# cornellius-gp/linear_operator

Measured on AMD Instinct MI355X. Metric: cg_member_matvecs_per_sec, higher is better.
Workload: dtype f32

## Files before the change

### linear_operator_amd/csrc/lo_rspace3.hip

```cpp
#include <algorithm>
#include <atomic>
#include <mutex>
#include <type_traits>
#include <stdlib.h>

#include "lo_device.h"
#include "lo_internal.h"
#include "lo_cg_onchip.h"
#include "lo_group_reduce.h"
#include "lo_cg_close.h"
#include "lo_f64_lanes.h"

namespace lo {

namespace {

typedef float f32x4 __attribute__((ext_vector_type(4)));
typedef __attribute__((address_space(1))) const f32x4 g_cf4;
typedef __attribute__((address_space(1))) const float g_cf;
typedef __attribute__((address_space(1))) float g_f;
typedef __attribute__((address_space(1))) const char g_cc;
template <class T>
__device__ __forceinline__ T* opaque_uniform(T* p) {
  asm volatile("" : "+s"(p));
  return p;
}

constexpr int R3_TPB = 256;
constexpr int R3_ROWS = 1024;

struct PeerOut {
  float* buf[7];
  int n;
  long long member_off;
};
PeerOut g_peer_out = {{nullptr, nullptr, nullptr, nullptr, nullptr, nullptr, nullptr}, 0, 0};
std::mutex g_peer_mu;

__host__ __device__ constexpr int r3_np(int RC) { return 2 * RC + 6; }

__device__ __forceinline__ unsigned xor4_dpp_u(unsigned x) {
  const int a = __builtin_amdgcn_update_dpp(0, (int)x, 0x104, 0xf, 0x5, false);
  return (unsigned)__builtin_amdgcn_update_dpp(a, (int)x, 0x114, 0xf, 0xa, false);
}
__device__ __forceinline__ double halve4_d(double lo, double hi, int lane) {
  const bool up = (lane & 4) != 0;
  const double keep = up ? hi : lo;
  const double send = up ? lo : hi;
  return keep + mk_d(xor4_dpp_u(lo_w(send)), xor4_dpp_u(hi_w(send)));
}

template <int CH>
__device__ __forceinline__ double rows_reduce_d(double (&p)[CH], int lane) {
  if constexpr (CH == 8) {
#pragma unroll
    for (int m = 0; m < 4; ++m) p[m] = halve4_d(p[m], p[m + 4], lane);
    p[0] = halve_pair_d<2>(p[0], p[2], lane);
    p[1] = halve_pair_d<2>(p[1], p[3], lane);
    return halve_pair_d<1>(p[0], p[1], lane);
  } else if constexpr (CH == 4) {
    p[0] = halve_pair_d<2>(p[0], p[2], lane);
    p[1] = halve_pair_d<2>(p[1], p[3], lane);
    return halve_pair_d<1>(p[0], p[1], lane);
  } else {
    return halve_pair_d<1>(p[0], p[1], lane);
  }
}

template <int RC, int GW>
__global__ __launch_bounds__(R3_TPB, 2) void k_cg_rspace3(OnchipArgs a, PeerOut po) {
  constexpr int CH = RC / 4;
  constexpr int RPI = 64 / CH;
  constexpr int NI = 256 / RPI;
  constexpr int NP = r3_np(RC);
  constexpr int MLD = RC + 2;
  constexpr int NH = RC / 2;
  constexpr int NG = 2 * GW * NP;
  __shared__ __attribute__((aligned(16))) float bst[4][256];
  __shared__ __attribute__((aligned(16))) float dst[4][256];
  __shared__ __attribute__((aligned(16))) double mat_s[3 * RC * MLD];
  __shared__ __attribute__((aligned(16))) double red[4][NP];
  __shared__ __attribute__((aligned(16))) double res[NP];
  __shared__ __attribute__((aligned(16))) double gv[4][32];
  __shared__ unsigned polw[GW > 1 ? NG : 2];
  const GroupPlace gp = group_place(GW, (int)gridDim.x / 8);
  if (!gp.active) return;
  const int grp = gp.grp, wig = gp.wig, ngroups = gp.ngroups;
  const int t = threadIdx.x, lane = t & 63, wave = t >> 6;
  const int wave_u = __builtin_amdgcn_readfirstlane(wave);
  unsigned long long* const gbase = a.gbuf + (size_t)grp * 2 * NG;
  unsigned tag = a.tag_base;
  bool same_xcd = false;
  const unsigned xcc = xcc_id();
  bool first = true;
  const int row0 = wig * R3_ROWS + 256 * wave_u;
  const int row0c = max(0, min(row0, a.N - 256));
  const bool di_full = a.dinv_mode == LO_DIAG_FULL;
  float* const bw = bst[wave_u];
  float* const dw = dst[wave_u];
  constexpr int NPF = 8;
  f32x4 pre[NPF];
  constexpr int NXT = NI - NPF;
  f32x4 nxt[NXT > 0 ? NXT : 1];
  auto request = [&](int64_t bm, int tl_, int i_lo, auto cnt, f32x4* dst) {
    const int ln_ = tl_ & 63, k_ = ln_ & (CH - 1), g_ = ln_ / CH;
    const unsigned loff = (unsigned)((g_ * RC + 4 * k_) * sizeof(float));
    g_cc* Cw = (g_cc*)(a.C + ((size_t)bm * a.N + row0c) * RC);
#pragma unroll
    for (int q = 0; q < decltype(cnt)::value / 8; ++q) {
      g_cc* bq = opaque_uniform(Cw + (i_lo + 8 * q + 4) * 1024);
#pragma unroll
      for (int i = 0; i < 8; ++i) dst[8 * q + i] = *(g_cf4*)(bq + loff + (i - 4) * 1024);
    }
  };
  int64_t b = grp;
  {
    int tl0 = t;
    asm volatile("" : "+v"(tl0));
    if (b < a.B) {
      request(b, tl0, 0, std::integral_constant<int, NPF>{}, pre);
      request(b, tl0, NPF, std::integral_constant<int, NXT>{}, nxt);
    } else {
#pragma unroll
      for (int i = 0; i < NPF; ++i) pre[i] = (f32x4){0.f, 0.f, 0.f, 0.f};
    }
  }
  while (b < a.B) {
    const bool stamp = a.dbg && b == a.dbg_member && wig == 0 && t == 0;
    if (stamp) a.dbg[0] = wall_clock64();
    int drawn = 0;
    if (wig == 0 && t == 0) drawn = atomicAdd(a.next_member, 1);
    int tl = t;
    asm volatile("" : "+v"(tl));
    const int ln = tl & 63, k = ln & (CH - 1), g = ln / CH;
    f32x4 Cr[NI];
#pragma unroll
    for (int i = 0; i < NPF; ++i) Cr[i] = pre[i];
#pragma unroll
    for (int i = 0; i < NXT; ++i) Cr[NPF + i] = nxt[i];
    float bq4[4], dq4[4];
    {
      g_cf* bb_ = opaque_uniform((g_cf*)(a.rhs + (size_t)b * a.N + row0c));
      g_cf* dd_ = opaque_uniform((g_cf*)(di_full ? a.dinv + (size_t)b * a.N + row0c : a.dinv + b));
      const int lo_e = row0 - row0c, hi_e = max(0, min(256, a.N - row0c));
      const int dstride = di_full ? 1 : 0;
#pragma unroll
      for (int m = 0; m < 4; ++m) {
        const int e = ln + 64 * m;
        const bool own = e >= lo_e && e < hi_e;
        bq4[m] = own ? bb_[e] : 0.f;
        dq4[m] = own ? dd_[e * dstride] : 0.f;
      }
    }
    constexpr int NM = (3 * RC * RC / 2 + R3_TPB - 1) / R3_TPB;
    f32x4 mv[NM];
    {
      typedef __attribute__((address_space(1))) const f32x4 g_m4;
      const g_m4* src = (const g_m4*)(a.RSD + (size_t)b * 6 * RC * RC);
#pragma unroll
      for (int u = 0; u < NM; ++u) {
        const int e = min(tl + R3_TPB * u, 3 * RC * RC / 2 - 1);
        const int ms = e / (RC * RC / 2);
        const int mg = ms == 0 ? 0 : ms + 1;
        mv[u] = src[(size_t)mg * (RC * RC / 2) + (e - ms * (RC * RC / 2))];
      }
    }
    const double lam_mine = a.RSD[((size_t)b * 6 + 5) * RC * RC + min(ln & 31, RC - 1)];
#pragma unroll
    for (int m = 0; m < 4; ++m) {
      bw[ln + 64 * m] = bq4[m];
      dw[ln + 64 * m] = dq4[m];
    }
#pragma unroll
    for (int u = 0; u < NM; ++u) {
      const int e = tl + R3_TPB * u;
      if (e < 3 * RC * RC / 2) {
        const int mi = e / (RC / 2), jj = e % (RC / 2);
        *reinterpret_cast<f32x4*>(&mat_s[mi * MLD + 2 * jj]) = mv[u];
      }
    }
    __builtin_amdgcn_wave_barrier();
    if (stamp) a.dbg[1] = wall_clock64();

    {
      double aw[4] = {0.0, 0.0, 0.0, 0.0}, au[4] = {0.0, 0.0, 0.0, 0.0};
#pragma unroll
      for (int i0 = 0; i0 < NI; i0 += 4) {
#pragma unroll
        for (int i = i0; i < i0 + 4; ++i) {
          const int r = RPI * i + g;
          const double bb = (double)bw[r];
          const double bd = bb * (double)dw[r];
          const double c0 = (double)Cr[i].x, c1 = (double)Cr[i].y, c2 = (double)Cr[i].z, c3 = (double)Cr[i].w;
          aw[0] = fma(c0, bd, aw[0]); au[0] = fma(c0, bb, au[0]);
          aw[1] = fma(c1, bd, aw[1]); au[1] = fma(c1, bb, au[1]);
          aw[2] = fma(c2, bd, aw[2]); au[2] = fma(c2, bb, au[2]);
          aw[3] = fma(c3, bd, aw[3]); au[3] = fma(c3, bb, au[3]);
        }
        __builtin_amdgcn_sched_barrier(0);
      }
      double s_acc = 0.0, a_acc = 0.0, d2_acc = 0.0;
#pragma unroll
      for (int j = 0; j < 4; ++j) {
        const int rw = 64 * j + RPI * k + g;
        const double bb = (double)bw[rw], di = (double)dw[rw];
        s_acc = fma(bb, bb * di, s_acc);
        a_acc = fma(bb, bb, a_acc);
        d2_acc = fma(di, di, d2_acc);
      }
      double h0 = halve_pair_d<32>(aw[0], au[0], ln), h1 = halve_pair_d<32>(aw[1], au[1], ln);
      double h2 = halve_pair_d<32>(aw[2], au[2], ln), h3 = halve_pair_d<32>(aw[3], au[3], ln);
      h0 = halve_pair_d<16>(h0, h2, ln);
      h1 = halve_pair_d<16>(h1, h3, ln);
      double mine = halve_pair_d<8>(h0, h1, ln);
      if constexpr (CH <= 4) mine = bfly_add_d<4>(mine);
      if constexpr (CH <= 2) mine = bfly_add_d<2>(mine);
      const int comp = (((ln >> 4) & 1) << 1) | ((ln >> 3) & 1);
      const bool writer = (ln & 7 & ~(CH - 1)) == 0;
      if (writer) red[wave_u][((ln >> 5) ? RC : 0) + 4 * k + comp] = mine;
      const double ssum = wave_sum_fast_d(s_acc), asum = wave_sum_fast_d(a_acc), d2sum = wave_sum_fast_d(d2_acc);
      if (ln == 0) {
        red[wave_u][2 * RC] = ssum;
        red[wave_u][2 * RC + 1] = asum;
        red[wave_u][2 * RC + 2] = (wig == 0 && wave_u == 0) ? (double)(ngroups + drawn) : 0.0;
        red[wave_u][2 * RC + 3] = d2sum;
        unsigned xc = xcc;
        asm volatile("" : "+s"(xc));
        red[wave_u][2 * RC + 4] = (first && wave_u == 0) ? (double)xc : 0.0;
        red[wave_u][2 * RC + 5] = (first && wave_u == 0) ? (double)(xc * xc) : 0.0;
      }
    }
#pragma unroll
    for (int i = 0; i < NI; ++i) asm volatile("" : "+v"(Cr[i]));
    __builtin_amdgcn_sched_barrier(0);
    if (a.prefetch & 4) __builtin_amdgcn_s_setprio(3);
    {
      ++tag;
      int tt = (int)threadIdx.x;
      asm volatile("" : "+v"(tt));
      __syncthreads();
      if constexpr (GW == 1) {
        if (tt < NP) res[tt] = (red[0][tt] + red[1][tt]) + (red[2][tt] + red[3][tt]);
      } else {
        unsigned long long* slot = gbase + (size_t)(tag & 1u) * NG;
        if (tt < NP) {
          const double v = (red[0][tt] + red[1][tt]) + (red[2][tt] + red[3][tt]);
          unsigned long long* mine = slot + ((size_t)wig * NP + tt) * 2;
          granule_store(mine, granule_pack_bits(tag, lo_w(v)), same_xcd);
          granule_store(mine + 1, granule_pack_bits(tag, hi_w(v)), same_xcd);
        }
        constexpr int PER = (NG + R3_TPB - 1) / R3_TPB;
        constexpr int CKQ = PER < 8 ? PER : 8;
        unsigned spin = 0;
        bool lost = false;
#pragma unroll 1
        for (int q0 = 0; q0 < PER && !lost; q0 += CKQ) {
          unsigned long long x[CKQ];
          for (;;) {
            bool ok = true;
#pragma unroll
            for (int q = 0; q < CKQ; ++q) {
              const int idx = tt + R3_TPB * (q0 + q);
              x[q] = granule_load(slot + min(idx, NG - 1));
              ok = ok && (granule_tag(x[q]) == tag);
            }
            if (ok) break;
            if (poll_give_up(spin, a.err)) {
              lost = true;
              break;
            }
            __builtin_amdgcn_s_sleep(1);
          }
#pragma unroll
          for (int q = 0; q < CKQ; ++q) {
            const int idx = tt + R3_TPB * (q0 + q);
            if (idx < NG) polw[idx] = granule_bits(x[q]);
          }
        }
        __syncthreads();
        if (tt < NP) {
          double tot = 0.0;
#pragma unroll
          for (int w = 0; w < GW; ++w) tot += mk_d(polw[(w * NP + tt) * 2], polw[(w * NP + tt) * 2 + 1]);
          res[tt] = tot;
        }
      }
      __syncthreads();
    }
    if (GW > 1 && first) {
      unsigned xc = xcc;
      asm volatile("" : "+s"(xc));
      same_xcd = same_xcd_verdict(res[2 * RC + 4], res[2 * RC + 5], GW, xc, a.allow_l2_handoff);
    }
    first = false;
    if (stamp) a.dbg[2] = wall_clock64();
    const int64_t b_next = (int64_t)res[2 * RC + 2];
    {
      int tp = t;
      asm volatile("" : "+v"(tp));
      if (b_next < a.B) {
        request(b_next, tp, 0, std::integral_constant<int, NPF>{}, pre);
      } else {
#pragma unroll
        for (int i = 0; i < NPF; ++i) pre[i] = (f32x4){0.f, 0.f, 0.f, 0.f};
      }
    }
    if (a.prefetch & 1) __builtin_amdgcn_s_setprio(3);

    const int j = lane & 31, hf = lane >> 5;
    const bool live = j < RC;
    const int jr = live ? j : RC - 1;
    double yj = 0.0, xi = 0.0;
    float nrm;
    {
      double a0 = res[2 * RC + 1], s = res[2 * RC];
      const double d2 = res[2 * RC + 3];
      nrm = sqrtf((float)a0);
      const bool rhs_zero = nrm < a.eps;
      if (rhs_zero) nrm = 1.0f;
      const double inv = 1.0 / (double)nrm;
      const double w0 = live ? res[jr] * inv : 0.0, u0 = live ? res[RC + jr] * inv : 0.0;
      s *= inv * inv;
      a0 *= inv * inv;
      float sa = a.stop_after;
      asm volatile("" : "+s"(sa));
      const double sure_rz = 2.0 * (double)sa * (double)sa * sqrt(d2);
      auto own_row_dot = [&](const double* mrow, const double* vec) {
        double a0_ = 0.0, a1_ = 0.0;
#pragma unroll
        for (int q = 0; q < NH; q += 2) {
          const double2 xa = *reinterpret_cast<const double2*>(mrow + q);
          const double2 xx = *reinterpret_cast<const double2*>(vec + q);
          a0_ = fma(xa.x, xx.x, a0_);
          a1_ = fma(xa.y, xx.y, a1_);
        }
        double lo_, up_;
        halves_d(a0_ + a1_, lo_, up_);
        return lo_ + up_;
      };
      double* myv = gv[wave];
      if (hf == 0) myv[j] = w0;
      __builtin_amdgcn_wave_barrier();
      const double* row0m = mat_s + (size_t)jr * MLD + hf * NH;
      double c0 = own_row_dot(row0m, myv + hf * NH);
      double e0 = own_row_dot(row0m + (size_t)1 * RC * MLD, myv + hf * NH);
      const double* nrow = row0m + (size_t)2 * RC * MLD;
      const double* tucol = mat_s + (size_t)(1 * RC + hf * NH) * MLD + jr;
      c0 = live ? c0 : 0.0;
      e0 = live ? e0 : 0.0;
      double tau2 = s - lanes32_sum_d(c0 * e0);
      tau2 = tau2 > 0.0 ? tau2 : 0.0;
      const bool delicate = !rhs_zero && tau2 < 1e-2 * s;
      const double lam = live ? lam_mine : 1.0;
      long long ts_a = 0, ts_b = 0;
      if (stamp) ts_a = wall_clock64();
      double cj = c0, qj = 0.0, etaj = 0.0;
      double cp = 1.0, qp = 0.0, etap = 0.0;
      double rz = 0.0, pApE = 0.0, alpha = 0.0, beta = 0.0;
      float rn = 0.f, last_alpha = 0.f;
      bool conv = false;
      unsigned close_flags = 0u;
      const size_t bc = (size_t)b;
      const bool rec = wig == 0 && lane == 0;
      const int last_owner = (a.iters - 1) & 3;
      for (int kk = -1; kk < a.iters; ++kk) {
        if (kk >= 0) {
          last_alpha = (float)alpha;
          etaj = fma(alpha, qj, etaj);
          etap = fma(alpha, qp, etap);
          cj = fma(-alpha * lam, qj, cj);
          cp = fma(-alpha, qp, cp);
        }
        const double lc = lam * cj;
        const bool lo_h = hf == 0;
        const float inv_rz = __builtin_amdgcn_rcpf((float)rz);
        const double red2 = row16_sum_d(halve_pair_d<16>(lo_h ? cj * cj : lc * qj, lo_h ? lc * cj : 0.0, lane));
        const auto pick = [&](double v, int ln_) {
          return mk_d((unsigned)__builtin_amdgcn_readlane((int)lo_w(v), ln_),
                      (unsigned)__builtin_amdgcn_readlane((int)hi_w(v), ln_));
        };
        const double cc = pick(red2, 0), clc = pick(red2, 16), clq = pick(red2, 32);
        const double rzn = fma(cp * cp, tau2, cc);
        const bool sure = rzn > sure_rz;
        const bool rec_first = kk == 0 && a.close_gran == nullptr && wave == 0;
        const bool rec_last = kk == a.iters - 1 && wave == last_owner;
        const bool own = rec_first || rec_last || !sure;
        float rnn = 0.f;
        if (kk < 0) {
          const float s1f = (float)a0;
          rnn = __builtin_amdgcn_sqrtf(s1f < 0.f ? 0.f : s1f);
        } else if (own) {
          const double dl = fma(-cp, c0, cj);
          __builtin_amdgcn_wave_barrier();
          if (hf == 0) myv[j] = dl;
          __builtin_amdgcn_wave_barrier();
          double gj_;
          {
            double a0_ = 0.0, a1_ = 0.0;
#pragma unroll
            for (int q = 0; q < NH; q += 2) {
              const double2 dd = *reinterpret_cast<const double2*>(myv + hf * NH + q);
              a0_ = fma(tucol[(size_t)q * MLD], dd.x, a0_);
              a1_ = fma(tucol[(size_t)(q + 1) * MLD], dd.y, a1_);
            }
            double lo_, up_;
            halves_d(a0_ + a1_, lo_, up_);
            gj_ = live ? lo_ + up_ : 0.0;
          }
          __builtin_amdgcn_wave_barrier();
          if (hf == 0) myv[j] = gj_;
          __builtin_amdgcn_wave_barrier();
          const double nd = own_row_dot(nrow, myv + hf * NH);
          const double r2 = row16_sum_d(halve_pair_d<16>(gj_ * nd, gj_ * u0, lane));
          const double dnd = pick(r2, 0), dm = pick(r2, 16);
          const double s1 = fma(cp, fma(cp, a0, 2.0 * dm), dnd);
          const float s1f = (float)s1;
          rnn = __builtin_amdgcn_sqrtf(s1f < 0.f ? 0.f : s1f);
        }
        if (kk >= 0) {
          beta = ((float)rz < a.eps) ? 0.0 : (double)((float)rzn * inv_rz);
          if (rhs_zero) rnn = 0.f;
          rn = rnn;
          if (rec && (rec_first || rec_last)) a.resid_rec[(size_t)kk * a.B + bc] = rn;
        } else {
          beta = 0.0;
          rn = rnn;
          if (wig == 0 && t == 0) a.init_conv[bc] = (rn < a.stop_after) ? 1 : 0;
          close_flags = ((rn < a.stop_after) ? 1u : 0u) | (delicate ? 4u : 0u);
          if (delicate && rec && wave == 0) atomicOr(a.err + 4, 1);
        }
        if (kk == 0 && (rnn != rnn || rzn != rzn)) close_flags |= 2u;
        conv = (own || rhs_zero) ? (rn < a.stop_after) : false;
        rz = rzn;
        pApE = fma(beta, fma(beta, pApE, 2.0 * clq), clc);
        qj = fma(beta, qj, cj);
        qp = fma(beta, qp, cp);
        const double pAp = fma(qp * qp, tau2, pApE);
        alpha = ((float)pAp < a.eps) ? 0.0 : (double)((float)rz * __builtin_amdgcn_rcpf((float)pAp));
        if (conv) alpha = 0.0;
      }
      if (stamp) ts_b = wall_clock64();
      if (rec && wave == last_owner) {
        a.rhs_norm[bc] = nrm;
        a.rhs_is_zero[bc] = rhs_zero ? 1 : 0;
        a.rz[bc] = (float)rz;
        a.alpha[bc] = last_alpha;
        a.beta[bc] = (float)beta;
        a.resid_norm[bc] = rn;
        a.has_conv[bc] = conv ? 1 : 0;
        if (a.close_gran) {
          granule_store(a.close_gran + b, granule_pack(a.close_epoch | close_flags, rn), false);
        }
      }
      __builtin_amdgcn_wave_barrier();
      if (hf == 0) myv[j] = fma(-etap, e0, etaj);
      __builtin_amdgcn_wave_barrier();
      xi = etap;
      {
        const double* col = mat_s + (size_t)(hf * NH) * MLD + jr;
        double a0_ = 0.0, a1_ = 0.0;
#pragma unroll
        for (int q = 0; q < NH; q += 2) {
          const double2 ee = *reinterpret_cast<const double2*>(myv + hf * NH + q);
          a0_ = fma(col[(size_t)q * MLD], ee.x, a0_);
          a1_ = fma(col[(size_t)(q + 1) * MLD], ee.y, a1_);
        }
        double lo_, up_;
        halves_d(a0_ + a1_, lo_, up_);
        yj = lo_ + up_;
      }
      yj = live ? yj : 0.0;
      if (stamp) {
        a.dbg[5] = ts_a - a.dbg[2];
        a.dbg[6] = ts_b - ts_a;
        a.dbg[7] = wall_clock64() - ts_b;
      }
      __builtin_amdgcn_wave_barrier();
      if (hf == 0) myv[j] = yj * (double)nrm;
      __builtin_amdgcn_wave_barrier();
    }
    if (!(a.prefetch & 2)) __builtin_amdgcn_s_setprio(0);
    if (stamp) a.dbg[3] = wall_clock64();
    {
      int l2 = lane;
      asm volatile("" : "+v"(l2));
      const int k2 = l2 & (CH - 1), g2 = l2 / CH;
      const double* myv = gv[wave];
      const double2 ya = *reinterpret_cast<const double2*>(&myv[4 * k2]);
      const double2 yb = *reinterpret_cast<const double2*>(&myv[4 * k2 + 2]);
      g_f* const xb = opaque_uniform((g_f*)(a.xout + (size_t)b * a.N + row0c));
      const bool more = b_next < a.B;
      g_cc* const Cn = (g_cc*)(a.C + ((size_t)(more ? b_next : b) * a.N + row0c) * RC);
      const unsigned loffn = (unsigned)((g2 * RC + 4 * k2) * sizeof(float));
#pragma unroll
      for (int js = 0; js < 4; ++js) {
        constexpr int J0 = NPF / CH;
        const int jj = (js + J0) & 3;
        double p[CH];
#pragma unroll
        for (int m = 0; m < CH; ++m) {
          const f32x4 c4 = Cr[CH * jj + m];
          p[m] = fma((double)c4.w, yb.y, fma((double)c4.z, yb.x, fma((double)c4.y, ya.y, (double)c4.x * ya.x)));
        }
        const double xv = rows_reduce_d<CH>(p, l2);
        const int rw = 64 * jj + RPI * k2 + g2;
        const int row = row0c + rw;
        const double acc = fma(xi, (double)bw[rw], xv);
        if (row >= row0 && row < a.N) {
          const float xval = (float)(acc * (double)dw[rw]);
          xb[rw] = xval;
          for (int pp = 0; pp < po.n; ++pp)
            ((g_f*)po.buf[pp])[((size_t)(b + po.member_off)) * a.N + row] = xval;
        }
        if (CH * jj >= NPF) {
          g_cc* bqn = opaque_uniform(Cn + (CH * jj + 4) * 1024);
#pragma unroll
          for (int m = 0; m < CH; ++m)
            nxt[CH * jj - NPF + m] = more ? *(g_cf4*)(bqn + loffn + (m - 4) * 1024) : (f32x4){0.f, 0.f, 0.f, 0.f};
        }
      }
      __builtin_amdgcn_wave_barrier();
    }
    __builtin_amdgcn_s_setprio(0);
    if (stamp) a.dbg[4] = wall_clock64();
    __syncthreads();
    b = b_next;
  }
  if (a.close_gran && wig == 0) cg_close_solve(a, ngroups, t);
}

int rspace3_prio() {
  static const int prio = [] {
    const char* e = getenv("LO_RS_PRIO");
    return e ? atoi(e) : 3;
  }();
  return prio;
}

constexpr size_t HO_MAX_WGS = 2 * 320;
constexpr size_t HO_GRAN_PER_WG = 432;
constexpr size_t HO_MAX_MEMBERS = 65536;
constexpr size_t HO_HEAD_BYTES = 256;
constexpr unsigned HO_TAG_LIMIT = 0xfff00000u;
constexpr unsigned HO_EPOCH_LIMIT = 0x1ffffff0u;
struct HandoffBlock {
  char* buf = nullptr;
  size_t bytes = 0;
  bool failed = false;
  unsigned next_tag = 1, next_epoch = 1;
  unsigned last_launch = 0;
  std::atomic<unsigned> confirmed{0};
  bool force_clear = false;
  unsigned clears = 0, launches = 0;
};
HandoffBlock g_handoff[16];
std::atomic<unsigned> g_handoff_ids{0};

HandoffBlock* handoff_block() {
  int dev = 0;
  if (hipGetDevice(&dev) != hipSuccess || dev < 0 || dev >= 16) return nullptr;
  HandoffBlock& h = g_handoff[dev];
  if (!h.buf && !h.failed) {
    h.bytes = HO_HEAD_BYTES + (HO_MAX_WGS * HO_GRAN_PER_WG + HO_MAX_MEMBERS) * sizeof(unsigned long long);
    if (hipMalloc(&h.buf, h.bytes) != hipSuccess || hipMemset(h.buf, 0, h.bytes) != hipSuccess) {
      (void)hipGetLastError();
      h.buf = nullptr;
      h.failed = true;
    }
  }
  return h.buf ? &h : nullptr;
}

bool handoff_advance(unsigned* next_tag, unsigned* next_epoch, int64_t B, unsigned* tag_base, unsigned* epoch) {
  bool wrap = false;
  const unsigned need = (unsigned)B + 2u;
  if (*next_tag >= HO_TAG_LIMIT - need || *next_epoch >= HO_EPOCH_LIMIT) {
    *next_tag = 1;
    *next_epoch = 1;
    wrap = true;
  }
  *tag_base = *next_tag;
  *epoch = *next_epoch;
  *next_tag += need;
  *next_epoch += 1;
  return wrap;
}

struct OwnedLaunch {
  bool inject;
  unsigned* launch_id;
};

template <int RC, int GW>
int rspace3_go(const OnchipArgs& a, int nwg, const OwnedLaunch* own, hipStream_t st) {
  int per_cu = 0;
  if (LO_OCCUPANCY_CACHED(per_cu, (k_cg_rspace3<RC, GW>), R3_TPB, 0) != hipSuccess || per_cu < 2) return LO_ERR_UNSUPPORTED;
  LO_PROF_BEGIN("cg_onchip", st);
  ResidentLaunch guard(st);
  OnchipArgs a2 = a;
  a2.prefetch = rspace3_prio();
  if (own) {
    hipStreamCaptureStatus cap = hipStreamCaptureStatusNone;
    if (hipStreamIsCapturing(st, &cap) != hipSuccess || cap != hipStreamCaptureStatusNone) {
      (void)hipGetLastError();
      return LO_ERR_UNSUPPORTED;
    }
    HandoffBlock* h = (a.B <= (int64_t)HO_MAX_MEMBERS && (size_t)2 * nwg <= HO_MAX_WGS) ? handoff_block() : nullptr;
    if (!h) return LO_ERR_UNSUPPORTED;
    bool clear = h->force_clear || h->last_launch != h->confirmed.load(std::memory_order_acquire);
    h->force_clear = false;
    clear = handoff_advance(&h->next_tag, &h->next_epoch, a.B, &a2.tag_base, &a2.close_epoch) || clear;
    h->last_launch = g_handoff_ids.fetch_add(1, std::memory_order_relaxed) + 1;
    if (h->last_launch == 0) h->last_launch = g_handoff_ids.fetch_add(1, std::memory_order_relaxed) + 1;
    *own->launch_id = h->last_launch;
    ++h->launches;
    if (clear) {
      ++h->clears;
      const int zrc = zero_span(h->buf, h->bytes, st);
      if (zrc) return zrc;
    }
    a2.close_epoch <<= 3;
    a2.handoff_owned = 1;
    a2.err = reinterpret_cast<int*>(h->buf);
    a2.next_member = a2.err + 1;
    a2.close_count = a2.err + 2;
    a2.gbuf = reinterpret_cast<unsigned long long*>(h->buf + HO_HEAD_BYTES);
    a2.close_gran = a2.gbuf + HO_MAX_WGS * HO_GRAN_PER_WG;
    if (own->inject) LO_HIP_CHECK(hipMemsetAsync(a2.err, 1, 1, st));
  }
  PeerOut po;
  {
    std::lock_guard<std::mutex> lk(g_peer_mu);
    po = g_peer_out;
  }
  hipLaunchKernelGGL((k_cg_rspace3<RC, GW>), dim3(2 * nwg), dim3(R3_TPB), 0, st, a2, po);
  LO_PROF_END(st);
  LO_LAUNCH_CHECK();
  return LO_OK;
}

template <int RC>
int rspace3_gw(const OnchipArgs& a, int nwg, const OwnedLaunch* own, hipStream_t st) {
  switch (a.GW) {
    case 1: return rspace3_go<RC, 1>(a, nwg, own, st);
    case 2: return rspace3_go<RC, 2>(a, nwg, own, st);
    case 4: return rspace3_go<RC, 4>(a, nwg, own, st);
    case 8: return rspace3_go<RC, 8>(a, nwg, own, st);
    case 16: return rspace3_go<RC, 16>(a, nwg, own, st);
    case 32: return rspace3_go<RC, 32>(a, nwg, own, st);
  }
  return LO_ERR_UNSUPPORTED;
}

int rspace3_dispatch(int RC, const OnchipArgs& a, int nwg, const OwnedLaunch* own, hipStream_t st) {
  if (!a.RSD || a.x || a.c != 1 || a.ab_rec || !a.xout || a.GW > 32 || a.N < 256 || (int64_t)a.GW * R3_ROWS < a.N)
    return LO_ERR_UNSUPPORTED;
  if (RC == 32) return rspace3_gw<32>(a, nwg, own, st);
  if (RC == 16) return rspace3_gw<16>(a, nwg, own, st);
  if (RC == 8) return rspace3_gw<8>(a, nwg, own, st);
  return LO_ERR_UNSUPPORTED;
}

}

int rspace3_launch(int RC, const OnchipArgs& a, int nwg, hipStream_t st) { return rspace3_dispatch(RC, a, nwg, nullptr, st); }

int rspace3_launch_owned(int RC, const OnchipArgs& a, int nwg, bool inject, unsigned* launch_id, hipStream_t st) {
  if (!a.close_gran || !a.close_ctrl || !a.close_mirror || a.dbg) return LO_ERR_UNSUPPORTED;
  const OwnedLaunch own = {inject, launch_id};
  return rspace3_dispatch(RC, a, nwg, &own, st);
}

void handoff_launch_confirm(unsigned launch_id) {
  int dev = 0;
  if (hipGetDevice(&dev) != hipSuccess || dev < 0 || dev >= 16) return;
  g_handoff[dev].confirmed.store(launch_id, std::memory_order_release);
}

}

extern "C" int lo_peer_gather_set(float* const* bufs, int n, long long member_offset) {
  if (n < 0 || n > 7 || (n > 0 && !bufs)) return LO_ERR_BADARG;
  std::lock_guard<std::mutex> lk(lo::g_peer_mu);
  for (int i = 0; i < 7; ++i) lo::g_peer_out.buf[i] = i < n ? bufs[i] : nullptr;
  lo::g_peer_out.n = n;
  lo::g_peer_out.member_off = member_offset;
  return LO_OK;
}

extern "C" int lo_resident_handoff_debug(int32_t force_clear, int64_t set_next_tag, int64_t set_next_epoch, uint32_t* out) {
  lo::ResidentLock guard;
  int dev = 0;
  if (hipGetDevice(&dev) != hipSuccess || dev < 0 || dev >= 16) return LO_ERR_BADARG;
  lo::HandoffBlock& h = lo::g_handoff[dev];
  if (set_next_tag > 0xffffffffll || set_next_epoch > 0xffffffffll) return LO_ERR_BADARG;
  if (set_next_tag >= 0) h.next_tag = (unsigned)set_next_tag;
  if (set_next_epoch >= 0) h.next_epoch = (unsigned)set_next_epoch;
  if (force_clear) h.force_clear = true;
  if (out) {
    out[0] = h.next_tag;
    out[1] = h.next_epoch;
    out[2] = h.clears;
    out[3] = h.launches;
  }
  return LO_OK;
}
```

Before: 36.68 million.

## Prefetch rhs/dinv into double-buffered LDS via direct global-to-LDS loads

Moves the per-member rhs and diagonal loads out of the critical path. They are now issued one member ahead with global_load_lds_dword into double-buffered shared arrays, and a vmcnt wait replaces the old synchronous register loads. The reduction-matrix loads are now issued after the C dot-product loop and stored to LDS during the cross-wave reduction, overlapping that latency. The member-draw atomic moves to the prefetch point. This adds LDS usage and depends on hand-written inline asm, with a fragile vmcnt count and careful m0 handling.

```diff
diff --git a/linear_operator_amd/csrc/lo_rspace3.hip b/linear_operator_amd/csrc/lo_rspace3.hip
--- a/linear_operator_amd/csrc/lo_rspace3.hip
+++ b/linear_operator_amd/csrc/lo_rspace3.hip
@@ -24,6 +24,18 @@
 __device__ __forceinline__ T* opaque_uniform(T* p) {
   asm volatile("" : "+s"(p));
   return p;
+}
+
+__device__ __forceinline__ void glds_dword(g_cf* base, unsigned voff, unsigned lds_dst) {
+  unsigned keep;
+  asm volatile(
+      "s_nop 4\n\ts_mov_b32 %0, m0\n\ts_mov_b32 m0, %3\n\ts_nop 0\n\tglobal_load_lds_dword %1, %2\n\ts_mov_b32 m0, %0"
+      : "=&s"(keep)
+      : "v"(voff), "s"(base), "s"(lds_dst)
+      : "memory");
+}
+__device__ __forceinline__ unsigned lds_addr(const float* p) {
+  return (unsigned)(size_t)(__attribute__((address_space(3))) const float*)p;
 }
 
 constexpr int R3_TPB = 256;
@@ -76,8 +88,8 @@
   constexpr int MLD = RC + 2;
   constexpr int NH = RC / 2;
   constexpr int NG = 2 * GW * NP;
-  __shared__ __attribute__((aligned(16))) float bst[4][256];
-  __shared__ __attribute__((aligned(16))) float dst[4][256];
+  __shared__ __attribute__((aligned(16))) float bst[2][4][256];
+  __shared__ __attribute__((aligned(16))) float dst[2][4][256];
   __shared__ __attribute__((aligned(16))) double mat_s[3 * RC * MLD];
   __shared__ __attribute__((aligned(16))) double red[4][NP];
   __shared__ __attribute__((aligned(16))) double res[NP];
@@ -96,8 +108,42 @@
   const int row0 = wig * R3_ROWS + 256 * wave_u;
   const int row0c = max(0, min(row0, a.N - 256));
   const bool di_full = a.dinv_mode == LO_DIAG_FULL;
-  float* const bw = bst[wave_u];
-  float* const dw = dst[wave_u];
+  auto stage_fill = [&](int64_t bm, int tl_, int par_) {
+    const int ln_ = tl_ & 63;
+    g_cf* bb_ = opaque_uniform((g_cf*)(a.rhs + (size_t)bm * a.N + row0c));
+    g_cf* dd_ = opaque_uniform((g_cf*)(di_full ? a.dinv + (size_t)bm * a.N + row0c : a.dinv + bm));
+    const int lo_e = row0 - row0c, hi_e = max(0, min(256, a.N - row0c));
+    const unsigned dstep = di_full ? 4u : 0u;
+    const unsigned lb = lds_addr(&bst[par_][wave_u][0]), ld = lds_addr(&dst[par_][wave_u][0]);
+#pragma unroll
+    for (int m = 0; m < 4; ++m) {
+      const int e = ln_ + 64 * m;
+      if (e >= lo_e && e < hi_e) {
+        glds_dword(bb_, 4u * (unsigned)e, lb + 256u * m);
+        glds_dword(dd_, dstep * (unsigned)e, ld + 256u * m);
+      }
+    }
+  };
+  {
+    const int lo_e = row0 - row0c, hi_e = max(0, min(256, a.N - row0c));
+#pragma unroll
+    for (int m = 0; m < 4; ++m) {
+      const int e = lane + 64 * m;
+      if (!(e >= lo_e && e < hi_e)) {
+        bst[0][wave_u][e] = 0.f; dst[0][wave_u][e] = 0.f;
+        bst[1][wave_u][e] = 0.f; dst[1][wave_u][e] = 0.f;
+      }
+    }
+  }
+  int drawn = 0;
+  auto draw = [&]() {
+    if (wig == 0 && t == 0) {
+      __attribute__((address_space(1))) int* nm = (__attribute__((address_space(1))) int*)a.next_member;
+      asm volatile("" : "+v"(nm));
+      drawn = __hip_atomic_fetch_add(nm, 1, __ATOMIC_RELAXED, __HIP_MEMORY_SCOPE_AGENT);
+    }
+  };
+  int par = 0;
   constexpr int NPF = 8;
   f32x4 pre[NPF];
   constexpr int NXT = NI - NPF;
@@ -118,6 +164,8 @@
     int tl0 = t;
     asm volatile("" : "+v"(tl0));
     if (b < a.B) {
+      stage_fill(b, tl0, 0);
+      draw();
       request(b, tl0, 0, std::integral_constant<int, NPF>{}, pre);
       request(b, tl0, NPF, std::integral_constant<int, NXT>{}, nxt);
     } else {
@@ -128,8 +176,8 @@
   while (b < a.B) {
     const bool stamp = a.dbg && b == a.dbg_member && wig == 0 && t == 0;
     if (stamp) a.dbg[0] = wall_clock64();
-    int drawn = 0;
-    if (wig == 0 && t == 0) drawn = atomicAdd(a.next_member, 1);
+    float* const bw = bst[par][wave_u];
+    float* const dw = dst[par][wave_u];
     int tl = t;
     asm volatile("" : "+v"(tl));
     const int ln = tl & 63, k = ln & (CH - 1), g = ln / CH;
@@ -138,23 +186,14 @@
     for (int i = 0; i < NPF; ++i) Cr[i] = pre[i];
 #pragma unroll
     for (int i = 0; i < NXT; ++i) Cr[NPF + i] = nxt[i];
-    float bq4[4], dq4[4];
-    {
-      g_cf* bb_ = opaque_uniform((g_cf*)(a.rhs + (size_t)b * a.N + row0c));
-      g_cf* dd_ = opaque_uniform((g_cf*)(di_full ? a.dinv + (size_t)b * a.N + row0c : a.dinv + b));
-      const int lo_e = row0 - row0c, hi_e = max(0, min(256, a.N - row0c));
-      const int dstride = di_full ? 1 : 0;
-#pragma unroll
-      for (int m = 0; m < 4; ++m) {
-        const int e = ln + 64 * m;
-        const bool own = e >= lo_e && e < hi_e;
-        bq4[m] = own ? bb_[e] : 0.f;
-        dq4[m] = own ? dd_[e * dstride] : 0.f;
-      }
-    }
+    asm volatile("s_waitcnt vmcnt(%0)" ::"n"(NI) : "memory");
+    __builtin_amdgcn_wave_barrier();
+    if (stamp) a.dbg[1] = wall_clock64();
+
     constexpr int NM = (3 * RC * RC / 2 + R3_TPB - 1) / R3_TPB;
     f32x4 mv[NM];
-    {
+    double lam_mine;
+    auto request_mats = [&]() {
       typedef __attribute__((address_space(1))) const f32x4 g_m4;
       const g_m4* src = (const g_m4*)(a.RSD + (size_t)b * 6 * RC * RC);
 #pragma unroll
@@ -164,24 +203,19 @@
         const int mg = ms == 0 ? 0 : ms + 1;
         mv[u] = src[(size_t)mg * (RC * RC / 2) + (e - ms * (RC * RC / 2))];
       }
-    }
-    const double lam_mine = a.RSD[((size_t)b * 6 + 5) * RC * RC + min(ln & 31, RC - 1)];
-#pragma unroll
-    for (int m = 0; m < 4; ++m) {
-      bw[ln + 64 * m] = bq4[m];
-      dw[ln + 64 * m] = dq4[m];
-    }
-#pragma unroll
-    for (int u = 0; u < NM; ++u) {
-      const int e = tl + R3_TPB * u;
-      if (e < 3 * RC * RC / 2) {
-        const int mi = e / (RC / 2), jj = e % (RC / 2);
-        *reinterpret_cast<f32x4*>(&mat_s[mi * MLD + 2 * jj]) = mv[u];
-      }
-    }
-    __builtin_amdgcn_wave_barrier();
-    if (stamp) a.dbg[1] = wall_clock64();
-
+      lam_mine = a.RSD[((size_t)b * 6 + 5) * RC * RC + min(ln & 31, RC - 1)];
+    };
+    auto store_mats = [&]() {
+#pragma unroll
+      for (int u = 0; u < NM; ++u) {
+        const int e = tl + R3_TPB * u;
+        if (e < 3 * RC * RC / 2) {
+          const int mi = e / (RC / 2), jj = e % (RC / 2);
+          *reinterpret_cast<f32x4*>(&mat_s[mi * MLD + 2 * jj]) = mv[u];
+        }
+      }
+      asm volatile("" : "+v"(lam_mine));
+    };
     {
       double aw[4] = {0.0, 0.0, 0.0, 0.0}, au[4] = {0.0, 0.0, 0.0, 0.0};
 #pragma unroll
@@ -199,6 +233,7 @@
         }
         __builtin_amdgcn_sched_barrier(0);
       }
+      request_mats();
       double s_acc = 0.0, a_acc = 0.0, d2_acc = 0.0;
 #pragma unroll
       for (int j = 0; j < 4; ++j) {
@@ -241,6 +276,7 @@
       __syncthreads();
       if constexpr (GW == 1) {
         if (tt < NP) res[tt] = (red[0][tt] + red[1][tt]) + (red[2][tt] + red[3][tt]);
+        store_mats();
       } else {
         unsigned long long* slot = gbase + (size_t)(tag & 1u) * NG;
         if (tt < NP) {
@@ -277,6 +313,7 @@
             if (idx < NG) polw[idx] = granule_bits(x[q]);
           }
         }
+        store_mats();
         __syncthreads();
         if (tt < NP) {
           double tot = 0.0;
@@ -299,6 +336,8 @@
       int tp = t;
       asm volatile("" : "+v"(tp));
       if (b_next < a.B) {
+        stage_fill(b_next, tp, par ^ 1);
+        draw();
         request(b_next, tp, 0, std::integral_constant<int, NPF>{}, pre);
       } else {
 #pragma unroll
@@ -491,7 +530,7 @@
       g_f* const xb = opaque_uniform((g_f*)(a.xout + (size_t)b * a.N + row0c));
       const bool more = b_next < a.B;
       g_cc* const Cn = (g_cc*)(a.C + ((size_t)(more ? b_next : b) * a.N + row0c) * RC);
-      const unsigned loffn = (unsigned)((g2 * RC + 4 * k2) * sizeof(float));
+      const unsigned loffn = more ? (unsigned)((g2 * RC + 4 * k2) * sizeof(float)) : 0u;
 #pragma unroll
       for (int js = 0; js < 4; ++js) {
         constexpr int J0 = NPF / CH;
@@ -515,8 +554,7 @@
         if (CH * jj >= NPF) {
           g_cc* bqn = opaque_uniform(Cn + (CH * jj + 4) * 1024);
 #pragma unroll
-          for (int m = 0; m < CH; ++m)
-            nxt[CH * jj - NPF + m] = more ? *(g_cf4*)(bqn + loffn + (m - 4) * 1024) : (f32x4){0.f, 0.f, 0.f, 0.f};
+          for (int m = 0; m < CH; ++m) nxt[CH * jj - NPF + m] = *(g_cf4*)(bqn + loffn + (m - 4) * 1024);
         }
       }
       __builtin_amdgcn_wave_barrier();
@@ -525,6 +563,7 @@
     if (stamp) a.dbg[4] = wall_clock64();
     __syncthreads();
     b = b_next;
+    par ^= 1;
   }
   if (a.close_gran && wig == 0) cg_close_solve(a, ngroups, t);
 }
```

New measurement: 36.63 million. About the same (-0.1%).
